# Alessandro-Mosconi/neptune-mip

Hardware: AMD Instinct MI355X
Metric: LP-relaxations/sec + objective gap vs reference, 512-node×256-function (higher is better)
Workload: dtype f32 x-state, f64 duals/reductions/certificate

## Files before the change

### include/neptune_lp.h

```cpp
#ifndef NEPTUNE_LP_H
#define NEPTUNE_LP_H

#include <stdint.h>

#ifdef __cplusplus
extern "C" {
#endif

#define NEP_API_VERSION 13

enum { NEP_MIN_DELAY = 0, NEP_MIN_UTILIZATION = 1, NEP_MIN_DELAY_AND_UTILIZATION = 2 };
enum { NEP_STEP1 = 1, NEP_STEP2_DELETE = 2, NEP_STEP2_CREATE = 3 };
enum { NEP_RELAX_REFERENCE = 0, NEP_RELAX_FACILITY = 1 };

enum { NEP_OK = 0, NEP_ERR_ARG = -1, NEP_ERR_HIP = -2, NEP_ERR_NOMEM = -3, NEP_ERR_STATE = -4 };

enum {
  NEP_LP_OPTIMAL = 0,
  NEP_LP_ITERATION_LIMIT = 1,
  NEP_LP_INFEASIBLE = 2,
  NEP_LP_CUTOFF = 3,
  NEP_LP_NUMERICAL = 4,
  NEP_LP_BOUND = 5
};
// ... 107 lines not shown
  NEP_SC_HANDLE_MAXDEV = 9,
  NEP_SC_CPU_MAXEXCESS = 10,
  NEP_SC_COUNT = 11
};
int nep_lp_score_check(void *model, int32_t slot, double *out);

int nep_get_stats(void *model, nep_stats *stats);

int nep_lp_get_diag(void *model, int32_t slot, double *out16);
int nep_debug_state(void *model, int32_t slot, double *y, double *kz, float *kty, double *lb, double *ub);
int nep_debug_sparse_rows(void *model, int32_t slot, int32_t *anchor_cnt, float *lambda_nnz);
int nep_debug_build(const nep_model_desc *desc, double *eta, double *rho, double *gam, double *rownorm,
                    int32_t *dims);
int nep_debug_presolve(const nep_model_desc *desc, int32_t n, const double *lb_int, const double *ub_int,
                       int32_t *ok_full, int32_t *ok_node, double *box_full, double *box_node);
void nep_reset_stats(void *model);

int nep_lp_copy_routing(void *dst_model, int32_t dst_slot, void *src_model, int32_t src_slot);

int nep_round_leaf(int32_t F, int32_t N, const double *c_fix, const double *n_fix, const float *flow, const double *zc,
                   const double *fn_mem, const double *node_mem, int32_t by_flow, double flow_threshold, double *c_out,
                   double *n_out);
int nep_round_leaves(int32_t F, int32_t N, const double *c_fix, const double *n_fix, const float *flow, const double *zc,
                     const double *fn_mem, const double *node_mem, int32_t modes, const int32_t *by_flow,
                     const double *flow_threshold, double *c_out, double *n_out, int32_t *found);

typedef struct {
  int32_t c0, c1, n0, n1, n_int;
  int32_t F, N;
  int32_t warm;
// ... 96 lines not shown
```

### neptune-mip_amd/core/engine/lp.py

```python
import ctypes
import math
import os

import numpy as np

_HERE = os.path.dirname(os.path.abspath(__file__))
LIB_PATH = os.environ.get("NEPTUNE_LP_LIB",
                          os.path.normpath(os.path.join(_HERE, "..", "..", "lib", "libneptune_lp.so")))

MIN_DELAY, MIN_UTILIZATION, MIN_DELAY_AND_UTILIZATION = 0, 1, 2
STEP1, STEP2_DELETE, STEP2_CREATE = 1, 2, 3
LP_OPTIMAL, LP_ITERATION_LIMIT, LP_INFEASIBLE, LP_CUTOFF, LP_NUMERICAL, LP_BOUND = 0, 1, 2, 3, 4, 5
VARIANTS = {"MinDelay": MIN_DELAY, "MinUtilization": MIN_UTILIZATION,
            "MinDelayAndUtilization": MIN_DELAY_AND_UTILIZATION}
API_VERSION = 13
RELAX_REFERENCE, RELAX_FACILITY = 0, 1

_dp = ctypes.POINTER(ctypes.c_double)


class EngineUnavailable(RuntimeError):
    pass


# ... 201 lines not shown
                               else BNB_RC_FIX())


EXPORTS = ("nep_model_create", "nep_model_destroy", "nep_model_get_info", "nep_lp_solve_batch",
           "nep_lp_submit", "nep_lp_submit_ex", "nep_lp_advance", "nep_lp_active", "nep_lp_copy_states", "nep_lp_get_flows_solutions",
           "nep_lp_get_solution", "nep_lp_get_rows", "nep_lp_copy_state", "nep_get_stats", "nep_reset_stats",
           "nep_lp_get_flows_split",
           "nep_last_error", "nep_api_version", "nep_lp_get_diag", "nep_debug_build", "nep_debug_state",
           "nep_debug_presolve", "nep_debug_sparse_rows", "nep_lp_set_params", "nep_lp_get_flows", "nep_lp_routing_entries",
           "nep_lp_allocation_entries", "nep_lp_score_check", "nep_round_leaf", "nep_lp_copy_routing",
           "nep_lp_get_solutions", "nep_round_leaves", "nep_lp_set_reference_weight",
           "nep_bnb_create", "nep_bnb_destroy", "nep_bnb_add_leaf", "nep_bnb_set_incumbent", "nep_bnb_event_data",
           "nep_bnb_run", "nep_bnb_get_stats", "nep_bnb_get_lp_iters", "nep_bnb_incumbent", "nep_bnb_set_step2",
           "nep_bnb_incumbent_event", "nep_bnb_debug_ibound", "nep_bnb_create_engines", "nep_bnb_sync_get",
           "nep_bnb_sync_set", "nep_bnb_export_nodes", "nep_bnb_import_nodes", "nep_lp_get_reduced_costs",
           "nep_lp_rc_fixings")
SCORE_FIELDS = ("network_delay", "nodes_used", "node_cost", "bad_c_x", "bad_memory", "bad_handle", "bad_cpu",
                "bad_n_c", "bad_budget", "handle_maxdev", "cpu_maxexcess")

_lib = None


def _host_inputs():
    return os.environ.get("NEP_HOST_INPUTS", "0") not in ("", "0")


def load_library(path=None):
    global _lib
    if _lib is not None and path is None:
        return _lib
    p = path or LIB_PATH
# ... 56 lines not shown
    lib.nep_bnb_sync_get.argtypes = [vp, _dp]
    lib.nep_bnb_sync_set.argtypes = [vp, ctypes.c_double, i32, i64]
    lib.nep_bnb_export_nodes.argtypes = [vp, i32, i32, pi32, _dp, pi32, _dp]
    lib.nep_bnb_import_nodes.argtypes = [vp, i32, pi32, _dp, pi32, _dp]
    lib.nep_lp_get_flows.argtypes = [vp, i32, pi32, ctypes.POINTER(ctypes.c_float)]
    lib.nep_lp_get_flows_split.argtypes = [vp, i32, pi32, ctypes.POINTER(ctypes.c_float), ctypes.POINTER(ctypes.c_float)]
    lib.nep_lp_routing_entries.argtypes = [vp, i32, ctypes.c_double, i32, i64, pi64, pi32, pi32, _dp]
    lib.nep_lp_allocation_entries.argtypes = [vp, i32, ctypes.c_double, i64, pi64, pi32, pi32]
    lib.nep_lp_score_check.argtypes = [vp, i32, _dp]
    lib.nep_round_leaf.argtypes = [i32, i32, _dp, _dp, ctypes.POINTER(ctypes.c_float), _dp, _dp, _dp, i32,
                                   ctypes.c_double, _dp, _dp]
    lib.nep_last_error.restype = ctypes.c_char_p
    lib.nep_api_version.restype = ctypes.c_int
    scalar_ptrs = tuple(ctypes.POINTER(t) for t in (ctypes.c_double, ctypes.c_float, ctypes.c_int32, ctypes.c_int64))
    for name in EXPORTS:
        fn = getattr(lib, name)
        if fn.argtypes:
            fn.argtypes = [ctypes.c_void_p if t in scalar_ptrs else t for t in fn.argtypes]
    if lib.nep_api_version() != API_VERSION:
        raise EngineUnavailable(f"{p}: API version {lib.nep_api_version()} != {API_VERSION} (rebuild the engine)")
    if path is None:
        _lib = lib
    return lib


def round_leaf(c_fix, n_fix, flow, zc, fn_mem, node_mem, by_flow, flow_threshold):
    lib = load_library()
    c_fix = np.ascontiguousarray(c_fix, np.float64)
    F, N = c_fix.shape
    nf = None if n_fix is None else np.ascontiguousarray(n_fix, np.float64)
# ... 84 lines not shown
    N, F = len(data.nodes), len(data.functions)
    v = VARIANTS[variant] if isinstance(variant, str) else int(variant)
    k = _arrays(data, N, F)
    d = _desc(k, N, F, v, int(step), alpha, soften_step1_sol, max_score, prev_network_delay, data.node_budget,
              relaxation)
    dims = np.zeros(4, np.int32)
    eta = np.zeros(1)
    _check(lib, lib.nep_debug_build(ctypes.byref(d), _ptr(eta), None, None, None, _ptr(dims, ctypes.c_int32)),
           "nep_debug_build")
    R, T, n_int, n_dual = dims.tolist()
    rho, gam, rn = np.zeros(n_dual), np.zeros(n_int), np.zeros(n_dual)
    _check(lib, lib.nep_debug_build(ctypes.byref(d), _ptr(eta), _ptr(rho), _ptr(gam), _ptr(rn), None),
           "nep_debug_build")
    return {"eta": float(eta[0]), "rho": rho, "gam": gam, "rownorm": rn, "R": R, "T": T, "n_int": n_int,
            "n_dual": n_dual}


def debug_presolve(data, variant, lb, ub, step=STEP1, alpha=0.5, soften_step1_sol=1.3, max_score=0.0,
                   prev_network_delay=0.0):
    lib = load_library()
    N, F = len(data.nodes), len(data.functions)
    v = VARIANTS[variant] if isinstance(variant, str) else int(variant)
    k = _arrays(data, N, F)
    d = _desc(k, N, F, v, int(step), alpha, soften_step1_sol, max_score, prev_network_delay, data.node_budget)
    lb = np.ascontiguousarray(lb, np.float64)
    ub = np.ascontiguousarray(ub, np.float64)
    n, ni = lb.shape
    okf = np.zeros(n, np.int32)
    okn = np.zeros(n, np.int32)
    bf = np.zeros((n, 2, ni))
# ... 287 lines not shown
```

### neptune-mip_amd/csrc/nep_fac.hip

```cpp
#include <hip/hip_runtime.h>
#include <cfloat>
#include <algorithm>
#include <cmath>

#include "nep_internal.h"
#include "nep_device.h"

namespace nep {

template <int CPL, bool CHECK, bool INIT, bool FIRST, int TW>
__global__ __launch_bounds__(kWave * TW) __attribute__((amdgpu_waves_per_eu(CHECK ? 2 : (CPL >= 8 ? 2 : (CPL >= 4 ? 3 : 4)), 8)))
void fac_x_pass(DeviceView v, const int32_t *__restrict__ slots, int plain, int it, int nslots, int nt_i) {
  const bool nt = nt_i != 0;
  constexpr int E = 4 * CPL;
  constexpr int SW = CHECK ? 2 : 1;
  extern __shared__ __attribute__((aligned(16))) float lds[];
  __shared__ double lds_s[TW][NTS + NBS];
  __shared__ double lds0[TW][4];
  const int total = v.F * nslots, Q = (total + 7) / 8;
  const int p = (int)(blockIdx.x % 8) * Q + (int)(blockIdx.x / 8);
  if (p >= total) return;
  const int f = p / nslots;
  const int slot = slots[p - f * nslots];
  Ctrl *ctrl = v.ctrl + slot;
// ... 524 lines not shown
    vals[BS_MOVE_Y] = a.mvy;
    vals[BS_DIST_Z] = a.dsz;
    vals[BS_DIST_Y] = a.dsy;
    vals[BS_LAGR0] = a.lagr0;
    double *bp = v.bpart + slot * v.sbpart + ((int64_t)F + jb) * NBS;
#pragma unroll
    for (int k = 0; k < NBS; ++k) {
      const double t = (k == BS_RES) ? wave_max_d(vals[k]) : wave_sum_d(vals[k]);
      if (lane == 0) bp[k] = t;
    }
  }
}

template <int CPL, int TW>
static hipError_t launch_fac_tw(const DeviceView &v, const int32_t *slots, int nslots, bool check, bool init,
                                bool first, bool plain, int it, hipStream_t s) {
  dim3 grid(8 * ((v.F * nslots + 7) / 8)), block(kWave * TW);
  const size_t lds = fac_lds_bytes(TW, v.NP, check);
  const int pl = plain ? 1 : 0;
  const int nt = (double)nslots * 4.0 * (double)v.sx * sizeof(float) > 160e6 ? 1 : 0;
  if (init) hipLaunchKernelGGL((fac_x_pass<CPL, false, true, false, TW>), grid, block, lds, s, v, slots, pl, it, nslots, nt);
  else if (check)
    hipLaunchKernelGGL((fac_x_pass<CPL, true, false, false, TW>), grid, block, lds, s, v, slots, pl, it, nslots, nt);
  else if (first)
    hipLaunchKernelGGL((fac_x_pass<CPL, false, false, true, TW>), grid, block, lds, s, v, slots, pl, it, nslots, nt);
  else hipLaunchKernelGGL((fac_x_pass<CPL, false, false, false, TW>), grid, block, lds, s, v, slots, pl, it, nslots, nt);
  return hipGetLastError();
}

static int fac_tile_waves(const DeviceView &v, int nslots, bool check) {
  int tw = 4;
  while (tw < 16 && (int64_t)nslots * v.F * tw < 4096) tw *= 2;
  if (v.CPL >= 4 && tw > 8) tw = 8;
  while (tw > kMinTileWaves && fac_lds_bytes(tw, v.NP, check) > kLdsCap) tw /= 2;
  return tw;
}

template <int CPL>
static hipError_t launch_fac_cpl(const DeviceView &v, const int32_t *slots, int nslots, bool check, bool init,
                                 bool first, bool plain, int it, hipStream_t s) {
  switch (fac_tile_waves(v, nslots, check)) {
    case 4: return launch_fac_tw<CPL, 4>(v, slots, nslots, check, init, first, plain, it, s);
    case 8: return launch_fac_tw<CPL, 8>(v, slots, nslots, check, init, first, plain, it, s);
    case 16: return launch_fac_tw<CPL, 16>(v, slots, nslots, check, init, first, plain, it, s);
    default: return hipErrorInvalidValue;
  }
}

hipError_t launch_fac_x_pass(const DeviceView &v, const int32_t *slots, int nslots, bool check, bool init, bool first,
                             bool plain, int it, hipStream_t s) {
  if (fac_lds_bytes(kMinTileWaves, v.NP, check) > kLdsCap) return hipErrorInvalidValue;
  switch (v.CPL) {
    case 1: return launch_fac_cpl<1>(v, slots, nslots, check, init, first, plain, it, s);
    case 2: return launch_fac_cpl<2>(v, slots, nslots, check, init, first, plain, it, s);
    case 4: return launch_fac_cpl<4>(v, slots, nslots, check, init, first, plain, it, s);
    case 8: return launch_fac_cpl<8>(v, slots, nslots, check, init, first, plain, it, s);
    default: return hipErrorInvalidValue;
  }
}

hipError_t launch_fac_node_pass(const DeviceView &v, const int32_t *slots, int nslots, bool check, bool init, bool first,
                                bool plain, int it, hipStream_t s) {
  const int fi = first ? 1 : 0, pl = plain ? 1 : 0;
  dim3 grid(v.JB, nslots), block(kNodeThreads);
  if (init) hipLaunchKernelGGL((fac_node_pass<false, true>), grid, block, 0, s, v, slots, fi, pl, it);
  else if (check) hipLaunchKernelGGL((fac_node_pass<true, false>), grid, block, 0, s, v, slots, fi, pl, it);
  else hipLaunchKernelGGL((fac_node_pass<false, false>), grid, block, 0, s, v, slots, fi, pl, it);
  return hipGetLastError();
}

}
// ... 1 lines not shown
```

### neptune-mip_amd/csrc/nep_host.cpp

```cpp
#include <hip/hip_runtime.h>

#include <algorithm>
#include <atomic>
#include <chrono>
#include <climits>
#include <cmath>
#include <cstdio>
#include <cstdlib>
#include <cstring>
#include <limits>
#include <memory>
#include <random>
#include <string>
#include <system_error>
#include <thread>
#include <vector>

#include "../../include/neptune_lp.h"
#include "nep_internal.h"

namespace nep {
hipError_t launch_x_pass(const DeviceView &v, const int32_t *slots, int nslots, bool check, bool init, bool first,
                         bool plain, int it, hipStream_t s);
hipError_t launch_node_pass(const DeviceView &v, const int32_t *slots, int nslots, bool check, bool init, bool first,
                            bool plain, int it, hipStream_t s);
hipError_t launch_scalar_pass(const DeviceView &v, const int32_t *slots, int nslots, bool check, bool init,
                              bool first, bool plain, int it, int block_len, hipStream_t s);
hipError_t launch_node_bounds(const DeviceView &v, const int32_t *slots, int nslots, const double *base_lb,
                              const double *base_ub, const uint8_t *base_mask, const int32_t *off, const int32_t *idx,
                              const double *cl, const double *cu, int max_chg, hipStream_t s);
hipError_t launch_init_slot(const DeviceView &v, const int32_t *slots, const int32_t *exact, int nslots, bool warm,
                            double eta, double omega0, const double *per, hipStream_t s);
hipError_t launch_node_flows(const DeviceView &v, const int32_t *slots, int n, float *out, float *wout,
                             hipStream_t s);
hipError_t launch_compact_f32(const float *vals, int rows, int cols, int64_t ld, double thr, int round3,
                              int32_t *cnt, int32_t *off, int32_t *orow, int32_t *ocol, double *oval, bool count_only,
                              hipStream_t s);
hipError_t launch_compact_f64(const double *vals, int rows, int cols, int64_t ld, double thr, int round3,
// ... 24 lines not shown
}
namespace nep {
int set_error(int code, const char *msg) { return fail(code, msg ? msg : ""); }
}
#define HIPCHK(expr)                                                                         \
  do {                                                                                       \
    hipError_t _e = (expr);                                                                  \
    if (_e != hipSuccess) return fail(NEP_ERR_HIP, std::string(#expr ": ") + hipGetErrorString(_e)); \
  } while (0)

static const double INF = std::numeric_limits<double>::infinity();
#ifndef NEP_HALPERN
#define NEP_HALPERN 1
#endif
static constexpr bool kHalpern = NEP_HALPERN != 0;

namespace {

struct Coo {
  std::vector<int> r, c;
  std::vector<double> v;
  void add(int row, int col, double val) {
    r.push_back(row);
    c.push_back(col);
    v.push_back(val);
  }
};

struct PresolveScratch {
  std::vector<int> pos, fdelta, touched, ftouched;
// ... 36 lines not shown
  bool score_x = false;
  std::vector<double> Dh;
  bool x_cost_free = true;
  bool base_ok = false;
  std::vector<double> base_lb, base_ub, base_amin, base_amax;
  std::vector<uint8_t> base_mask;
  std::vector<int> base_cnt, Kcp, Kcr;
  std::vector<double> Kcv;
  std::vector<PresolveScratch> psc;
  double eta = 0, sigma_max = 0, omega0 = 1.0;
  double omega_ref = 0.0;
  hipStream_t stream = nullptr;
  bool own_stream = false;
  hipStream_t aux = nullptr;
  hipEvent_t ev_aux = nullptr;
  DeviceView v{};
  std::vector<void *> allocs;
  double *d_prm = nullptr;
  double prm_host[3] = {0, 0, 0};
  bool prm_sent = false;
  int32_t *d_slots = nullptr;
  int32_t *h_act = nullptr;
  int32_t *d_new = nullptr;
  double *d_base_lb = nullptr, *d_base_ub = nullptr;
  uint8_t *d_base_mask = nullptr;
  int32_t *d_sub_i = nullptr;
  double *d_sub_d = nullptr;
  hipEvent_t ev0 = nullptr, ev1 = nullptr;
  nep_stats stats{};
  float *d_flows = nullptr;
// ... 22 lines not shown
  double *h_rc = nullptr;
  double *d_rc = nullptr;
  int32_t *d_rccnt = nullptr, *d_rcoff = nullptr;
  int32_t *d_rcidx = nullptr;
  double *d_rcval = nullptr;
  std::vector<uint8_t> rc_stale;
  int32_t *h_sub_i[2] = {nullptr, nullptr};
  double *h_sub_d[2] = {nullptr, nullptr};
  size_t cap_sub_i[2] = {0, 0}, cap_sub_d[2] = {0, 0};
  hipEvent_t ev_sub[2] = {nullptr, nullptr};
  bool sub_pending[2] = {false, false};
  int sub_k = 0;
  ~Model() {
    if (stream) (void)hipStreamSynchronize(stream);
    if (aux) (void)hipStreamSynchronize(aux);
    if (h_ctrl) (void)hipHostFree(h_ctrl);
    if (h_act) (void)hipHostFree(h_act);
    if (h_flows) (void)hipHostFree(h_flows);
    if (h_sols) (void)hipHostFree(h_sols);
    if (h_rc) (void)hipHostFree(h_rc);
    for (int k = 0; k < 2; ++k) {
      if (h_sub_i[k]) (void)hipHostFree(h_sub_i[k]);
      if (h_sub_d[k]) (void)hipHostFree(h_sub_d[k]);
      if (ev_sub[k]) (void)hipEventDestroy(ev_sub[k]);
    }
    for (void *p : allocs) (void)hipFree(p);
    for (hipGraphExec_t g : block_graph)
      if (g) (void)hipGraphExecDestroy(g);
    if (ev0) (void)hipEventDestroy(ev0);
    if (ev1) (void)hipEventDestroy(ev1);
    if (ev_aux) (void)hipEventDestroy(ev_aux);
    if (aux) (void)hipStreamDestroy(aux);
    if (own_stream && stream) (void)hipStreamDestroy(stream);
  }
};

template <typename T>
int dalloc(Model &m, T **p, size_t n) {
  void *q = nullptr;
  if (n == 0) n = 1;
  hipError_t e = hipMalloc(&q, n * sizeof(T));
  if (e != hipSuccess) return fail(NEP_ERR_NOMEM, std::string("hipMalloc: ") + hipGetErrorString(e));
  m.allocs.push_back(q);
  *p = static_cast<T *>(q);
  return NEP_OK;
}
template <typename T>
// ... 20 lines not shown
  if (d.step != NEP_STEP1 && !d.old_allocations) return fail(NEP_ERR_ARG, "step 2 needs old_allocations");
  m.N = N;
  m.F = F;
  m.variant = d.variant;
  m.step = d.step;
  m.step2 = d.step != NEP_STEP1;
  m.has_n = d.variant != NEP_MIN_DELAY;
  if (d.relaxation != NEP_RELAX_REFERENCE && d.relaxation != NEP_RELAX_FACILITY) return fail(NEP_ERR_ARG, "bad relaxation");
  m.fac = d.relaxation == NEP_RELAX_FACILITY;
  if (m.fac && (m.step2 || !m.has_n))
    return fail(NEP_ERR_ARG, "the facility relaxation is a step-1 MinUtilization / MinDelayAndUtilization model");
  m.alpha = d.alpha;
  m.M = d.big_m > 0 ? d.big_m : 1e6;
  m.eps = d.epsilon > 0 ? d.epsilon : 1e-6;
  m.sigma4 = d.step == NEP_STEP2_CREATE ? 1.0 : -1.0;
  m.NP = (N + 3) / 4 * 4;
  if (const int np_max = max_padded_width(m.fac); m.NP > np_max)
    return fail(NEP_ERR_ARG, "n_nodes = " + std::to_string(N) + " not supported by this build: the " +
                                 (m.fac ? "facility" : "reference") + " relaxation's certificate pass holds rows of at most " +
                                 std::to_string(np_max) + " destinations in LDS (largest supported n_nodes: " +
                                 std::to_string(np_max) + ")");
  const int chunks = m.NP / 4;
  m.CPL = chunks <= 64 ? 1 : chunks <= 128 ? 2 : chunks <= 256 ? 4 : 8;
  m.W.assign(d.workload, d.workload + (size_t)F * N);
  m.cprh.assign(d.core_per_req, d.core_per_req + (size_t)F * N);
  m.wsum.assign(F, 0.0);
  for (int f = 0; f < F; ++f)
    for (int i = 0; i < N; ++i) m.wsum[f] += m.W[(size_t)f * N + i];
  const double *D = d.delay;

  for (int f = 0; f < F; ++f) {
    int zeros = 0;
    for (int i = 0; i < N; ++i) {
      const double w = m.W[(size_t)f * N + i];
      if (w != 0.0) {
        m.row_f.push_back(f);
        m.row_src.push_back(i);
        m.row_m.push_back(1.f);
// ... 414 lines not shown
    m.stream = (hipStream_t)stream;
  } else {
    HIPCHK(hipStreamCreateWithFlags(&m.stream, hipStreamNonBlocking));
    m.own_stream = true;
  }
  HIPCHK(hipEventCreate(&m.ev0));
  HIPCHK(hipEventCreate(&m.ev1));
  {
    int least = 0, greatest = 0;
    if (hipDeviceGetStreamPriorityRange(&least, &greatest) != hipSuccess) greatest = 0;
    const char *e = std::getenv("NEP_AUX_PRIORITY");
    if (e && std::atoi(e) == 0) greatest = least;
    HIPCHK(hipStreamCreateWithPriority(&m.aux, hipStreamNonBlocking, greatest));
  }
  HIPCHK(hipEventCreateWithFlags(&m.ev_aux, hipEventDisableTiming));
  DeviceView &v = m.v;
  v.N = m.N; v.NP = m.NP; v.F = m.F; v.R = m.R; v.JB = m.JB; v.CPL = m.CPL;
  v.has_n = m.has_n; v.step2 = m.step2; v.variant = m.variant; v.fac = m.fac;
  v.M = m.M; v.eps = m.eps; v.sigma4 = m.sigma4; v.cost_n = m.cost_n; v.score_n_coef = m.score_n_coef;
  v.w_dis = m.w_dis;
  v.dred = m.dred; v.sT = m.sT; v.sum_old = m.sum_old;
  v.dl = m.dl; v.il = m.il;
  v.rs_suff = 0.2; v.rs_nec = 0.9; v.rs_art = 0.36; v.omega_smooth = 0.5;
  if (const char *e = std::getenv("NEP_RESTART")) std::sscanf(e, "%lf,%lf,%lf", &v.rs_suff, &v.rs_nec, &v.rs_art);
  if (const char *e = std::getenv("NEP_OMEGA_SMOOTH")) v.omega_smooth = std::atof(e);
  if (const char *e = std::getenv("NEP_PIPELINE_MAX_DONE")) m.pipe_max_done = std::atoi(e);
  v.polish_res = kPolishRes;
  v.polish_budget = kPolishBudget;
  if (const char *e = std::getenv("NEP_POLISH")) {
    long long b = v.polish_budget;
// ... 718 lines not shown
  double *dlb = m.d_sub_d, *dub = dlb + nchg;
  HIPCHK(hipEventRecord(m.ev_sub[sk], m.aux));
  HIPCHK(launch_node_bounds(v, dn, nf, m.d_base_lb, m.d_base_ub, m.d_base_mask, doff, didx, dlb, dub, max_chg,
                            m.aux));
  HIPCHK(launch_init_slot(v, dn, dex, nf, o.warm_start != 0, m.eta, m.omega0, per ? dub + nchg : nullptr, m.aux));
  HIPCHK(launch_x_pass(v, dn, nf, false, true, true, true, 0, m.aux));
  HIPCHK(launch_node_pass(v, dn, nf, false, true, true, true, 0, m.aux));
  HIPCHK(launch_scalar_pass(v, dn, nf, false, true, true, true, 0, o.check_every, m.aux));
  HIPCHK(hipEventRecord(m.ev_aux, m.aux));
  HIPCHK(hipStreamWaitEvent(m.stream, m.ev_aux, 0));
  m.act.insert(m.act.end(), fresh.begin(), fresh.end());
  m.sub_pending[sk] = true;
  return NEP_OK;
}

hipError_t block_graph(Model &m, int na, hipGraphExec_t *out) {
  const int ce = m.run.check_every;
  if (m.graph_ce != ce) {
    for (hipGraphExec_t &g : m.block_graph)
      if (g) { (void)hipGraphExecDestroy(g); g = nullptr; }
    m.block_graph.assign(m.max_batch + 1, nullptr);
    m.graph_ce = ce;
  }
  if (!m.block_graph[na]) {
    hipError_t e = hipStreamBeginCapture(m.stream, hipStreamCaptureModeThreadLocal);
    if (e != hipSuccess) return e;
    hipError_t le = hipSuccess;
    for (int it = 0; it < ce && le == hipSuccess; ++it) {
      const bool check = it == 0, first = it == 1;
      const bool plain = !kHalpern || ce < 4 || it == 0 || it == ce - 1;
      le = launch_x_pass(m.v, m.d_slots, na, check, false, first, plain, it, m.stream);
      if (le == hipSuccess) le = launch_node_pass(m.v, m.d_slots, na, check, false, first, plain, it, m.stream);
      if (le == hipSuccess && (m.step2 || check))
        le = launch_scalar_pass(m.v, m.d_slots, na, check, false, first, plain, it, ce, m.stream);
    }
    hipGraph_t graph = nullptr;
    e = hipStreamEndCapture(m.stream, &graph);
    if (le != hipSuccess) { if (graph) (void)hipGraphDestroy(graph); return le; }
    if (e != hipSuccess) return e;
    hipGraphExec_t exec = nullptr;
    e = hipGraphInstantiate(&exec, graph, nullptr, nullptr, 0);
    (void)hipGraphDestroy(graph);
    if (e != hipSuccess) return e;
    m.block_graph[na] = exec;
  }
  *out = m.block_graph[na];
  return hipSuccess;
}

int launch_block(Model &m) {
  DeviceView &v = m.v;
  const int ce = m.run.check_every;
  const int na = (int)m.act.size();
  const int sample_it = (ce >= 4 && m.blocks % 4 == 0) ? 2 : -1;
  m.blocks += 1;
  std::copy(m.act.begin(), m.act.end(), m.h_act);
  HIPCHK(hipMemcpyAsync(m.d_slots, m.h_act, na * sizeof(int32_t), hipMemcpyHostToDevice, m.stream));
  bool eager = sample_it >= 0 || !m.graphs_ok;
  if (!eager) {
    hipGraphExec_t g = nullptr;
    if (block_graph(m, na, &g) != hipSuccess) {
      (void)hipGetLastError();
      m.graphs_ok = false;
      eager = true;
    } else {
      HIPCHK(hipGraphLaunch(g, m.stream));
      m.stats.x_pass_launches += ce;
    }
  }
  for (int it = 0; it < ce && eager; ++it) {
    const bool check = it == 0, first = it == 1;
    const bool plain = !kHalpern || ce < 4 || it == 0 || it == ce - 1;
    const bool sample = it == sample_it;
    if (sample) HIPCHK(hipEventRecord(m.ev0, m.stream));
    HIPCHK(launch_x_pass(v, m.d_slots, na, check, false, first, plain, it, m.stream));
    if (sample) HIPCHK(hipEventRecord(m.ev1, m.stream));
    HIPCHK(launch_node_pass(v, m.d_slots, na, check, false, first, plain, it, m.stream));
    if (m.step2 || check) HIPCHK(launch_scalar_pass(v, m.d_slots, na, check, false, first, plain, it, ce, m.stream));
    m.stats.x_pass_launches += 1;
  }
  HIPCHK(hipMemcpyAsync(m.h_ctrl, v.ctrl, sizeof(Ctrl) * m.max_batch, hipMemcpyDeviceToHost, m.stream));
  m.stats.lp_iterations += (int64_t)na * ce;
  m.launched = m.act;
  m.inflight = true;
  m.inflight_sampled = sample_it >= 0;
  return NEP_OK;
}

int advance(Model &m, int min_done, int32_t *n_done, int32_t *done, double *obj, double *pobj, int32_t *status,
            int64_t *iters) {
  *n_done = 0;
  while (true) {
    if (!m.inflight) {
      if (m.act.empty()) break;
      int rc = launch_block(m);
// ... 735 lines not shown
  if (!desc) return fail(NEP_ERR_ARG, "null argument");
  if (desc->device_inputs) return fail(NEP_ERR_ARG, "nep_debug_build takes host arrays (device_inputs = 0)");
  Model m;
  int rc = build(m, *desc);
  if (rc) return rc;
  if (eta) *eta = m.eta;
  if (rho) std::memcpy(rho, m.rho.data(), m.rho.size() * sizeof(double));
  if (gam) std::memcpy(gam, m.gam.data(), m.gam.size() * sizeof(double));
  if (rownorm) std::memcpy(rownorm, m.rownorm.data(), m.rownorm.size() * sizeof(double));
  if (dims) {
    dims[0] = m.R; dims[1] = m.F; dims[2] = m.il.n_int; dims[3] = m.dl.n_dual;
  }
  return NEP_OK;
}

int nep_get_stats(void *model, nep_stats *stats) {
  if (!model || !stats) return fail(NEP_ERR_ARG, "null argument");
  *stats = static_cast<Model *>(model)->stats;
  return NEP_OK;
}

void nep_reset_stats(void *model) {
  if (model) static_cast<Model *>(model)->stats = nep_stats{};
}

}

int nep_debug_presolve(const nep_model_desc *desc, int32_t n, const double *lbi, const double *ubi, int32_t *ok_full,
                       int32_t *ok_node, double *box_full, double *box_node) {
  if (!desc || n < 0 || !ok_full || !ok_node) return fail(NEP_ERR_ARG, "null argument");
// ... 38 lines not shown
```

### neptune-mip_amd/csrc/nep_internal.h

```cpp
#pragma once
#include <cstddef>
#include <cstdint>

#ifndef NEP_NT
#define NEP_NT 1
#endif
#ifndef NEP_SPARSE_ANCHOR
#define NEP_SPARSE_ANCHOR 1
#endif
#ifndef NEP_INLINE_REFLECT
#define NEP_INLINE_REFLECT 0
#endif

#if defined(__HIPCC__) || defined(__HIP__)
#define NEP_HD __host__ __device__
#else
#define NEP_HD
#endif

namespace nep {

NEP_HD inline void dred_interval(double sigma4, double la, double ua, double ld, double ud, double &tlo, double &thi) {
  if (sigma4 > 0) {
    const bool ok = ld <= 0.0 && ud >= 0.0;
// ... 15 lines not shown
  int32_t j;
  float v;
};

constexpr int kWave = 64;

constexpr size_t kLdsCap = 144 * 1024;
constexpr int kMinTileWaves = 4;
NEP_HD inline size_t x_lds_bytes(int tw, int NP, bool check) {
  return (size_t)(2 * tw + 2) * NP * sizeof(float) +
         (check ? (size_t)(NEP_INLINE_REFLECT ? 3 : 2) * tw * NP * sizeof(float) + 4 * (size_t)NP * sizeof(double) : 0);
}
NEP_HD inline size_t fac_lds_bytes(int tw, int NP, bool check) {
  const int sw = check ? 2 : 1;
  return (size_t)(sw * tw + tw + (check ? tw : 0) + 3) * NP * sizeof(float) + 3 * (size_t)NP * sizeof(double);
}
inline int max_padded_width(bool fac) {
  int np = 4;
  while ((fac ? fac_lds_bytes(kMinTileWaves, np + 4, true) : x_lds_bytes(kMinTileWaves, np + 4, true)) <= kLdsCap) np += 4;
  return np;
}

constexpr int64_t kOmegaTrained = 1024;
constexpr double kPolishRes = 1e-3;
constexpr int64_t kPolishBudget = 512;
constexpr int kNodeWaves = 16;
constexpr int kNodeThreads = kWave * kNodeWaves;
constexpr int kNodeJ = 16;

struct RowInfo {
// ... 119 lines not shown
```

### neptune-mip_amd/csrc/nep_kernels.hip

```cpp
#include <hip/hip_runtime.h>
#include <cfloat>
#include <algorithm>
#include <cmath>

#include "nep_internal.h"
#include "nep_device.h"

#ifndef NEP_XPASS_PREFETCH
#define NEP_XPASS_PREFETCH 2
#endif
#ifndef NEP_CHECK_WAVES
#define NEP_CHECK_WAVES 2
#endif
#ifndef NEP_XPASS_WAVES
#define NEP_XPASS_WAVES 6
#endif
#ifndef NEP_XPASS_PF_WAVES
#define NEP_XPASS_PF_WAVES 5
#endif
#ifndef NEP_XPASS_PF_ANCHOR
#define NEP_XPASS_PF_ANCHOR 0
#endif
#ifndef NEP_XPASS_ELIDE
#define NEP_XPASS_ELIDE 1
// ... 1351 lines not shown
  uint8_t *mask = v.mask + slot * v.smask;
  const int oc = v.il.oc, FN = v.F * v.N;
  for (int t = off[b] + blockIdx.x * blockDim.x + threadIdx.x; t < off[b + 1]; t += gridDim.x * blockDim.x) {
    const int k = idx[t];
    lb[k] = cl[t];
    ub[k] = cu[t];
    if (k >= oc && k < oc + FN) {
      const int f = (k - oc) / v.N, j = (k - oc) - f * v.N;
      mask[(int64_t)f * v.NP + j] = cu[t] > 0.0 ? 1 : 0;
    }
  }
}

template <int CPL, int TW>
static hipError_t launch_x_tw(const DeviceView &v, const int32_t *slots, int nslots, bool check, bool init,
                              bool first, bool plain, int it, hipStream_t s) {
  dim3 grid(8 * ((v.F * nslots + 7) / 8)), block(kWave * TW);
  const size_t lds = x_lds_bytes(TW, v.NP, check);
  const int pl = plain ? 1 : 0;
  const int nt = (double)nslots * 2.0 * (double)v.sx * sizeof(float) > 160e6 ? 1 : 0;
  if (init) hipLaunchKernelGGL((x_pass<CPL, false, true, false, TW>), grid, block, lds, s, v, slots, pl, it, nslots, nt);
  else if (check)
    hipLaunchKernelGGL((x_pass<CPL, true, false, false, TW>), grid, block, lds, s, v, slots, pl, it, nslots, nt);
  else if (first)
    hipLaunchKernelGGL((x_pass<CPL, false, false, true, TW>), grid, block, lds, s, v, slots, pl, it, nslots, nt);
  else hipLaunchKernelGGL((x_pass<CPL, false, false, false, TW>), grid, block, lds, s, v, slots, pl, it, nslots, nt);
  return hipGetLastError();
}

static int tile_waves(const DeviceView &v, int nslots, bool check) {
  int tw = 4;
  while (tw < 16 && (int64_t)nslots * v.F * tw < 4096) tw *= 2;
  if (v.CPL >= 8 && tw > 8) tw = 8;
  while (check && tw > kMinTileWaves && x_lds_bytes(tw, v.NP, true) > kLdsCap) tw /= 2;
  return tw;
}

template <int CPL>
static hipError_t launch_x_cpl(const DeviceView &v, const int32_t *slots, int nslots, bool check, bool init,
                               bool first, bool plain, int it, hipStream_t s) {
  switch (tile_waves(v, nslots, check)) {
    case 4: return launch_x_tw<CPL, 4>(v, slots, nslots, check, init, first, plain, it, s);
    case 8: return launch_x_tw<CPL, 8>(v, slots, nslots, check, init, first, plain, it, s);
    case 16: return launch_x_tw<CPL, 16>(v, slots, nslots, check, init, first, plain, it, s);
    default: return hipErrorInvalidValue;
  }
}

hipError_t launch_fac_x_pass(const DeviceView &v, const int32_t *slots, int nslots, bool check, bool init, bool first,
                             bool plain, int it, hipStream_t s);
hipError_t launch_fac_node_pass(const DeviceView &v, const int32_t *slots, int nslots, bool check, bool init, bool first,
                                bool plain, int it, hipStream_t s);

hipError_t launch_x_pass(const DeviceView &v, const int32_t *slots, int nslots, bool check, bool init, bool first,
                         bool plain, int it, hipStream_t s) {
  if (v.fac) return launch_fac_x_pass(v, slots, nslots, check, init, first, plain, it, s);
  if (x_lds_bytes(kMinTileWaves, v.NP, check) > kLdsCap) return hipErrorInvalidValue;
  switch (v.CPL) {
    case 1: return launch_x_cpl<1>(v, slots, nslots, check, init, first, plain, it, s);
    case 2: return launch_x_cpl<2>(v, slots, nslots, check, init, first, plain, it, s);
    case 4: return launch_x_cpl<4>(v, slots, nslots, check, init, first, plain, it, s);
    case 8: return launch_x_cpl<8>(v, slots, nslots, check, init, first, plain, it, s);
    default: return hipErrorInvalidValue;
  }
}

hipError_t launch_node_pass(const DeviceView &v, const int32_t *slots, int nslots, bool check, bool init, bool first,
                            bool plain, int it, hipStream_t s) {
  if (v.fac) return launch_fac_node_pass(v, slots, nslots, check, init, first, plain, it, s);
  const int fi = first ? 1 : 0, pl = plain ? 1 : 0;
  dim3 grid(v.JB, nslots), block(kNodeThreads);
  if (init) hipLaunchKernelGGL((node_pass<false, true>), grid, block, 0, s, v, slots, fi, pl, it);
  else if (check) hipLaunchKernelGGL((node_pass<true, false>), grid, block, 0, s, v, slots, fi, pl, it);
  else hipLaunchKernelGGL((node_pass<false, false>), grid, block, 0, s, v, slots, fi, pl, it);
  return hipGetLastError();
}

// ... 33 lines not shown
```

Baseline: 17.17.

## Split each LP block batch into two stream groups that run concurrently

Splits the active LP slots of each iteration block into two halves and launches the x/node/scalar pass chains for each half on separate streams, joined by fork/join events and captured into the block graph. Because the halves have no dependencies on each other, their kernel chains can overlap instead of running behind per-iteration serialization of the whole batch. The split only happens when both halves keep the same tile-wave choice, and the non-temporal store policy still uses the full batch size. It adds stream and event setup, falls back to a single group if graph capture fails, and comes with a debug export for checking the split decision.

```diff
diff --git a/include/neptune_lp.h b/include/neptune_lp.h
--- a/include/neptune_lp.h
+++ b/include/neptune_lp.h
@@ -145,6 +145,7 @@
                     int32_t *dims);
 int nep_debug_presolve(const nep_model_desc *desc, int32_t n, const double *lb_int, const double *ub_int,
                        int32_t *ok_full, int32_t *ok_node, double *box_full, double *box_node);
+int nep_debug_block_split(int32_t n_nodes, int32_t n_functions, int32_t relaxation, int32_t na, int32_t *out3);
 void nep_reset_stats(void *model);
 
 int nep_lp_copy_routing(void *dst_model, int32_t dst_slot, void *src_model, int32_t src_slot);
diff --git a/neptune-mip_amd/core/engine/lp.py b/neptune-mip_amd/core/engine/lp.py
--- a/neptune-mip_amd/core/engine/lp.py
+++ b/neptune-mip_amd/core/engine/lp.py
@@ -239,7 +239,7 @@
            "nep_bnb_run", "nep_bnb_get_stats", "nep_bnb_get_lp_iters", "nep_bnb_incumbent", "nep_bnb_set_step2",
            "nep_bnb_incumbent_event", "nep_bnb_debug_ibound", "nep_bnb_create_engines", "nep_bnb_sync_get",
            "nep_bnb_sync_set", "nep_bnb_export_nodes", "nep_bnb_import_nodes", "nep_lp_get_reduced_costs",
-           "nep_lp_rc_fixings")
+           "nep_lp_rc_fixings", "nep_debug_block_split")
 SCORE_FIELDS = ("network_delay", "nodes_used", "node_cost", "bad_c_x", "bad_memory", "bad_handle", "bad_cpu",
                 "bad_n_c", "bad_budget", "handle_maxdev", "cpu_maxexcess")
 
@@ -326,6 +326,8 @@
     lib.nep_api_version.restype = ctypes.c_int
     scalar_ptrs = tuple(ctypes.POINTER(t) for t in (ctypes.c_double, ctypes.c_float, ctypes.c_int32, ctypes.c_int64))
     for name in EXPORTS:
+        if name == "nep_debug_block_split":
+            continue
         fn = getattr(lib, name)
         if fn.argtypes:
             fn.argtypes = [ctypes.c_void_p if t in scalar_ptrs else t for t in fn.argtypes]
@@ -440,6 +442,15 @@
            "nep_debug_build")
     return {"eta": float(eta[0]), "rho": rho, "gam": gam, "rownorm": rn, "R": R, "T": T, "n_int": n_int,
             "n_dual": n_dual}
+
+
+def debug_block_split(n_nodes, n_functions, na, relaxation=RELAX_REFERENCE):
+    lib = load_library()
+    lib.nep_debug_block_split.argtypes = [ctypes.c_int32] * 4 + [ctypes.c_void_p]
+    out = np.zeros(3, np.int32)
+    _check(lib, lib.nep_debug_block_split(int(n_nodes), int(n_functions), int(relaxation), int(na),
+                                          _ptr(out, ctypes.c_int32)), "nep_debug_block_split")
+    return tuple(int(t) for t in out)
 
 
 def debug_presolve(data, variant, lb, ub, step=STEP1, alpha=0.5, soften_step1_sol=1.3, max_score=0.0,
diff --git a/neptune-mip_amd/csrc/nep_fac.hip b/neptune-mip_amd/csrc/nep_fac.hip
--- a/neptune-mip_amd/csrc/nep_fac.hip
+++ b/neptune-mip_amd/csrc/nep_fac.hip
@@ -562,11 +562,11 @@
 
 template <int CPL, int TW>
 static hipError_t launch_fac_tw(const DeviceView &v, const int32_t *slots, int nslots, bool check, bool init,
-                                bool first, bool plain, int it, hipStream_t s) {
+                                bool first, bool plain, int it, hipStream_t s, int policy_slots) {
   dim3 grid(8 * ((v.F * nslots + 7) / 8)), block(kWave * TW);
   const size_t lds = fac_lds_bytes(TW, v.NP, check);
   const int pl = plain ? 1 : 0;
-  const int nt = (double)nslots * 4.0 * (double)v.sx * sizeof(float) > 160e6 ? 1 : 0;
+  const int nt = (double)policy_slots * 4.0 * (double)v.sx * sizeof(float) > 160e6 ? 1 : 0;
   if (init) hipLaunchKernelGGL((fac_x_pass<CPL, false, true, false, TW>), grid, block, lds, s, v, slots, pl, it, nslots, nt);
   else if (check)
     hipLaunchKernelGGL((fac_x_pass<CPL, true, false, false, TW>), grid, block, lds, s, v, slots, pl, it, nslots, nt);
@@ -586,23 +586,25 @@
 
 template <int CPL>
 static hipError_t launch_fac_cpl(const DeviceView &v, const int32_t *slots, int nslots, bool check, bool init,
-                                 bool first, bool plain, int it, hipStream_t s) {
+                                 bool first, bool plain, int it, hipStream_t s, int policy_slots) {
   switch (fac_tile_waves(v, nslots, check)) {
-    case 4: return launch_fac_tw<CPL, 4>(v, slots, nslots, check, init, first, plain, it, s);
-    case 8: return launch_fac_tw<CPL, 8>(v, slots, nslots, check, init, first, plain, it, s);
-    case 16: return launch_fac_tw<CPL, 16>(v, slots, nslots, check, init, first, plain, it, s);
+    case 4: return launch_fac_tw<CPL, 4>(v, slots, nslots, check, init, first, plain, it, s, policy_slots);
+    case 8: return launch_fac_tw<CPL, 8>(v, slots, nslots, check, init, first, plain, it, s, policy_slots);
+    case 16: return launch_fac_tw<CPL, 16>(v, slots, nslots, check, init, first, plain, it, s, policy_slots);
     default: return hipErrorInvalidValue;
   }
 }
 
+int fac_block_tile_waves(const DeviceView &v, int nslots, bool check) { return fac_tile_waves(v, nslots, check); }
+
 hipError_t launch_fac_x_pass(const DeviceView &v, const int32_t *slots, int nslots, bool check, bool init, bool first,
-                             bool plain, int it, hipStream_t s) {
+                             bool plain, int it, hipStream_t s, int policy_slots) {
   if (fac_lds_bytes(kMinTileWaves, v.NP, check) > kLdsCap) return hipErrorInvalidValue;
   switch (v.CPL) {
-    case 1: return launch_fac_cpl<1>(v, slots, nslots, check, init, first, plain, it, s);
-    case 2: return launch_fac_cpl<2>(v, slots, nslots, check, init, first, plain, it, s);
-    case 4: return launch_fac_cpl<4>(v, slots, nslots, check, init, first, plain, it, s);
-    case 8: return launch_fac_cpl<8>(v, slots, nslots, check, init, first, plain, it, s);
+    case 1: return launch_fac_cpl<1>(v, slots, nslots, check, init, first, plain, it, s, policy_slots);
+    case 2: return launch_fac_cpl<2>(v, slots, nslots, check, init, first, plain, it, s, policy_slots);
+    case 4: return launch_fac_cpl<4>(v, slots, nslots, check, init, first, plain, it, s, policy_slots);
+    case 8: return launch_fac_cpl<8>(v, slots, nslots, check, init, first, plain, it, s, policy_slots);
     default: return hipErrorInvalidValue;
   }
 }
diff --git a/neptune-mip_amd/csrc/nep_host.cpp b/neptune-mip_amd/csrc/nep_host.cpp
--- a/neptune-mip_amd/csrc/nep_host.cpp
+++ b/neptune-mip_amd/csrc/nep_host.cpp
@@ -21,7 +21,9 @@
 
 namespace nep {
 hipError_t launch_x_pass(const DeviceView &v, const int32_t *slots, int nslots, bool check, bool init, bool first,
-                         bool plain, int it, hipStream_t s);
+                         bool plain, int it, hipStream_t s, int policy_slots = 0);
+int block_tile_waves(const DeviceView &v, int nslots, bool check);
+int block_split(const DeviceView &v, int na);
 hipError_t launch_node_pass(const DeviceView &v, const int32_t *slots, int nslots, bool check, bool init, bool first,
                             bool plain, int it, hipStream_t s);
 hipError_t launch_scalar_pass(const DeviceView &v, const int32_t *slots, int nslots, bool check, bool init,
@@ -76,6 +78,7 @@
 #define NEP_HALPERN 1
 #endif
 static constexpr bool kHalpern = NEP_HALPERN != 0;
+static constexpr int kBlockGroups = 2;
 
 namespace {
 
@@ -142,6 +145,9 @@
   bool own_stream = false;
   hipStream_t aux = nullptr;
   hipEvent_t ev_aux = nullptr;
+  hipStream_t grp = nullptr;
+  hipEvent_t ev_fork = nullptr, ev_join = nullptr;
+  int groups = 1;
   DeviceView v{};
   std::vector<void *> allocs;
   double *d_prm = nullptr;
@@ -194,6 +200,7 @@
   ~Model() {
     if (stream) (void)hipStreamSynchronize(stream);
     if (aux) (void)hipStreamSynchronize(aux);
+    if (grp) (void)hipStreamSynchronize(grp);
     if (h_ctrl) (void)hipHostFree(h_ctrl);
     if (h_act) (void)hipHostFree(h_act);
     if (h_flows) (void)hipHostFree(h_flows);
@@ -211,6 +218,9 @@
     if (ev1) (void)hipEventDestroy(ev1);
     if (ev_aux) (void)hipEventDestroy(ev_aux);
     if (aux) (void)hipStreamDestroy(aux);
+    if (ev_fork) (void)hipEventDestroy(ev_fork);
+    if (ev_join) (void)hipEventDestroy(ev_join);
+    if (grp) (void)hipStreamDestroy(grp);
     if (own_stream && stream) (void)hipStreamDestroy(stream);
   }
 };
@@ -261,14 +271,13 @@
   m.M = d.big_m > 0 ? d.big_m : 1e6;
   m.eps = d.epsilon > 0 ? d.epsilon : 1e-6;
   m.sigma4 = d.step == NEP_STEP2_CREATE ? 1.0 : -1.0;
-  m.NP = (N + 3) / 4 * 4;
+  m.NP = padded_width(N);
   if (const int np_max = max_padded_width(m.fac); m.NP > np_max)
     return fail(NEP_ERR_ARG, "n_nodes = " + std::to_string(N) + " not supported by this build: the " +
                                  (m.fac ? "facility" : "reference") + " relaxation's certificate pass holds rows of at most " +
                                  std::to_string(np_max) + " destinations in LDS (largest supported n_nodes: " +
                                  std::to_string(np_max) + ")");
-  const int chunks = m.NP / 4;
-  m.CPL = chunks <= 64 ? 1 : chunks <= 128 ? 2 : chunks <= 256 ? 4 : 8;
+  m.CPL = chunks_per_lane(m.NP);
   m.W.assign(d.workload, d.workload + (size_t)F * N);
   m.cprh.assign(d.core_per_req, d.core_per_req + (size_t)F * N);
   m.wsum.assign(F, 0.0);
@@ -713,6 +722,13 @@
     HIPCHK(hipStreamCreateWithPriority(&m.aux, hipStreamNonBlocking, greatest));
   }
   HIPCHK(hipEventCreateWithFlags(&m.ev_aux, hipEventDisableTiming));
+  m.groups = kBlockGroups;
+  if (const char *e = std::getenv("NEP_BLOCK_GROUPS")) m.groups = std::atoi(e) >= 2 ? 2 : 1;
+  if (m.groups > 1) {
+    HIPCHK(hipStreamCreateWithFlags(&m.grp, hipStreamNonBlocking));
+    HIPCHK(hipEventCreateWithFlags(&m.ev_fork, hipEventDisableTiming));
+    HIPCHK(hipEventCreateWithFlags(&m.ev_join, hipEventDisableTiming));
+  }
   DeviceView &v = m.v;
   v.N = m.N; v.NP = m.NP; v.F = m.F; v.R = m.R; v.JB = m.JB; v.CPL = m.CPL;
   v.has_n = m.has_n; v.step2 = m.step2; v.variant = m.variant; v.fac = m.fac;
@@ -1461,26 +1477,48 @@
   return NEP_OK;
 }
 
-hipError_t block_graph(Model &m, int na, hipGraphExec_t *out) {
+hipError_t launch_iters(Model &m, const int32_t *slots, int n, int na, int it0, int it1, hipStream_t s) {
+  const int ce = m.run.check_every;
+  hipError_t e = hipSuccess;
+  for (int it = it0; it < it1 && e == hipSuccess; ++it) {
+    const bool check = it == 0, first = it == 1;
+    const bool plain = !kHalpern || ce < 4 || it == 0 || it == ce - 1;
+    e = launch_x_pass(m.v, slots, n, check, false, first, plain, it, s, na);
+    if (e == hipSuccess) e = launch_node_pass(m.v, slots, n, check, false, first, plain, it, s);
+    if (e == hipSuccess && (m.step2 || check)) e = launch_scalar_pass(m.v, slots, n, check, false, first, plain, it, ce, s);
+  }
+  return e;
+}
+
+hipError_t launch_span(Model &m, int na, int nA, int it0, int it1) {
+  if (it0 >= it1) return hipSuccess;
+  if (!nA) return launch_iters(m, m.d_slots, na, na, it0, it1, m.stream);
+  hipError_t e = hipEventRecord(m.ev_fork, m.stream);
+  if (e == hipSuccess) e = hipStreamWaitEvent(m.grp, m.ev_fork, 0);
+  if (e != hipSuccess) return e;
+  const hipError_t ea = launch_iters(m, m.d_slots, nA, na, it0, it1, m.stream);
+  const hipError_t eb = launch_iters(m, m.d_slots + nA, na - nA, na, it0, it1, m.grp);
+  e = hipEventRecord(m.ev_join, m.grp);
+  if (e == hipSuccess) e = hipStreamWaitEvent(m.stream, m.ev_join, 0);
+  return ea != hipSuccess ? ea : eb != hipSuccess ? eb : e;
+}
+
+void drop_block_graphs(Model &m) {
+  for (hipGraphExec_t &g : m.block_graph)
+    if (g) { (void)hipGraphExecDestroy(g); g = nullptr; }
+  m.block_graph.assign(m.max_batch + 1, nullptr);
+}
+
+hipError_t block_graph(Model &m, int na, int nA, hipGraphExec_t *out) {
   const int ce = m.run.check_every;
   if (m.graph_ce != ce) {
-    for (hipGraphExec_t &g : m.block_graph)
-      if (g) { (void)hipGraphExecDestroy(g); g = nullptr; }
-    m.block_graph.assign(m.max_batch + 1, nullptr);
+    drop_block_graphs(m);
     m.graph_ce = ce;
   }
   if (!m.block_graph[na]) {
     hipError_t e = hipStreamBeginCapture(m.stream, hipStreamCaptureModeThreadLocal);
     if (e != hipSuccess) return e;
-    hipError_t le = hipSuccess;
-    for (int it = 0; it < ce && le == hipSuccess; ++it) {
-      const bool check = it == 0, first = it == 1;
-      const bool plain = !kHalpern || ce < 4 || it == 0 || it == ce - 1;
-      le = launch_x_pass(m.v, m.d_slots, na, check, false, first, plain, it, m.stream);
-      if (le == hipSuccess) le = launch_node_pass(m.v, m.d_slots, na, check, false, first, plain, it, m.stream);
-      if (le == hipSuccess && (m.step2 || check))
-        le = launch_scalar_pass(m.v, m.d_slots, na, check, false, first, plain, it, ce, m.stream);
-    }
+    const hipError_t le = launch_span(m, na, nA, 0, ce);
     hipGraph_t graph = nullptr;
     e = hipStreamEndCapture(m.stream, &graph);
     if (le != hipSuccess) { if (graph) (void)hipGraphDestroy(graph); return le; }
@@ -1503,29 +1541,40 @@
   m.blocks += 1;
   std::copy(m.act.begin(), m.act.end(), m.h_act);
   HIPCHK(hipMemcpyAsync(m.d_slots, m.h_act, na * sizeof(int32_t), hipMemcpyHostToDevice, m.stream));
+  int nA = m.groups > 1 ? block_split(v, na) : 0;
   bool eager = sample_it >= 0 || !m.graphs_ok;
   if (!eager) {
     hipGraphExec_t g = nullptr;
-    if (block_graph(m, na, &g) != hipSuccess) {
+    hipError_t e = block_graph(m, na, nA, &g);
+    if (e != hipSuccess && nA) {
+      (void)hipGetLastError();
+      m.groups = 1;
+      nA = 0;
+      drop_block_graphs(m);
+      e = block_graph(m, na, 0, &g);
+    }
+    if (e != hipSuccess) {
       (void)hipGetLastError();
       m.graphs_ok = false;
       eager = true;
     } else {
       HIPCHK(hipGraphLaunch(g, m.stream));
-      m.stats.x_pass_launches += ce;
-    }
-  }
-  for (int it = 0; it < ce && eager; ++it) {
-    const bool check = it == 0, first = it == 1;
-    const bool plain = !kHalpern || ce < 4 || it == 0 || it == ce - 1;
-    const bool sample = it == sample_it;
-    if (sample) HIPCHK(hipEventRecord(m.ev0, m.stream));
-    HIPCHK(launch_x_pass(v, m.d_slots, na, check, false, first, plain, it, m.stream));
-    if (sample) HIPCHK(hipEventRecord(m.ev1, m.stream));
-    HIPCHK(launch_node_pass(v, m.d_slots, na, check, false, first, plain, it, m.stream));
-    if (m.step2 || check) HIPCHK(launch_scalar_pass(v, m.d_slots, na, check, false, first, plain, it, ce, m.stream));
-    m.stats.x_pass_launches += 1;
-  }
+    }
+  }
+  if (eager) {
+    const int s0 = sample_it >= 0 ? sample_it : ce, s1 = sample_it >= 0 ? sample_it + 1 : ce;
+    HIPCHK(launch_span(m, na, nA, 0, s0));
+    if (sample_it >= 0) {
+      const bool plain = !kHalpern;
+      HIPCHK(hipEventRecord(m.ev0, m.stream));
+      HIPCHK(launch_x_pass(v, m.d_slots, na, false, false, false, plain, sample_it, m.stream));
+      HIPCHK(hipEventRecord(m.ev1, m.stream));
+      HIPCHK(launch_node_pass(v, m.d_slots, na, false, false, false, plain, sample_it, m.stream));
+      if (m.step2) HIPCHK(launch_scalar_pass(v, m.d_slots, na, false, false, false, plain, sample_it, ce, m.stream));
+    }
+    HIPCHK(launch_span(m, na, nA, s1, ce));
+  }
+  m.stats.x_pass_launches += ce;
   HIPCHK(hipMemcpyAsync(m.h_ctrl, v.ctrl, sizeof(Ctrl) * m.max_batch, hipMemcpyDeviceToHost, m.stream));
   m.stats.lp_iterations += (int64_t)na * ce;
   m.launched = m.act;
@@ -2291,6 +2340,21 @@
   return NEP_OK;
 }
 
+int nep_debug_block_split(int32_t n_nodes, int32_t n_functions, int32_t relaxation, int32_t na, int32_t *out3) {
+  if (!out3 || n_nodes < 1 || n_functions < 1 || na < 1) return fail(NEP_ERR_ARG, "bad argument");
+  DeviceView v{};
+  v.N = n_nodes;
+  v.F = n_functions;
+  v.fac = relaxation == NEP_RELAX_FACILITY ? 1 : 0;
+  v.NP = padded_width(n_nodes);
+  if (v.NP > max_padded_width(v.fac != 0)) return fail(NEP_ERR_ARG, "n_nodes beyond the widest supported row");
+  v.CPL = chunks_per_lane(v.NP);
+  out3[0] = block_split(v, na);
+  out3[1] = block_tile_waves(v, na, false);
+  out3[2] = block_tile_waves(v, na, true);
+  return NEP_OK;
+}
+
 int nep_get_stats(void *model, nep_stats *stats) {
   if (!model || !stats) return fail(NEP_ERR_ARG, "null argument");
   *stats = static_cast<Model *>(model)->stats;
diff --git a/neptune-mip_amd/csrc/nep_internal.h b/neptune-mip_amd/csrc/nep_internal.h
--- a/neptune-mip_amd/csrc/nep_internal.h
+++ b/neptune-mip_amd/csrc/nep_internal.h
@@ -53,6 +53,11 @@
 NEP_HD inline size_t fac_lds_bytes(int tw, int NP, bool check) {
   const int sw = check ? 2 : 1;
   return (size_t)(sw * tw + tw + (check ? tw : 0) + 3) * NP * sizeof(float) + 3 * (size_t)NP * sizeof(double);
+}
+inline int padded_width(int N) { return (N + 3) / 4 * 4; }
+inline int chunks_per_lane(int NP) {
+  const int chunks = NP / 4;
+  return chunks <= 64 ? 1 : chunks <= 128 ? 2 : chunks <= 256 ? 4 : 8;
 }
 inline int max_padded_width(bool fac) {
   int np = 4;
diff --git a/neptune-mip_amd/csrc/nep_kernels.hip b/neptune-mip_amd/csrc/nep_kernels.hip
--- a/neptune-mip_amd/csrc/nep_kernels.hip
+++ b/neptune-mip_amd/csrc/nep_kernels.hip
@@ -1389,11 +1389,11 @@
 
 template <int CPL, int TW>
 static hipError_t launch_x_tw(const DeviceView &v, const int32_t *slots, int nslots, bool check, bool init,
-                              bool first, bool plain, int it, hipStream_t s) {
+                              bool first, bool plain, int it, hipStream_t s, int policy_slots) {
   dim3 grid(8 * ((v.F * nslots + 7) / 8)), block(kWave * TW);
   const size_t lds = x_lds_bytes(TW, v.NP, check);
   const int pl = plain ? 1 : 0;
-  const int nt = (double)nslots * 2.0 * (double)v.sx * sizeof(float) > 160e6 ? 1 : 0;
+  const int nt = (double)policy_slots * 2.0 * (double)v.sx * sizeof(float) > 160e6 ? 1 : 0;
   if (init) hipLaunchKernelGGL((x_pass<CPL, false, true, false, TW>), grid, block, lds, s, v, slots, pl, it, nslots, nt);
   else if (check)
     hipLaunchKernelGGL((x_pass<CPL, true, false, false, TW>), grid, block, lds, s, v, slots, pl, it, nslots, nt);
@@ -1411,31 +1411,48 @@
   return tw;
 }
 
+int fac_block_tile_waves(const DeviceView &v, int nslots, bool check);
+
+int block_tile_waves(const DeviceView &v, int nslots, bool check) {
+  return v.fac ? fac_block_tile_waves(v, nslots, check) : tile_waves(v, nslots, check);
+}
+
+int block_split(const DeviceView &v, int na) {
+  if (na < 2) return 0;
+  const int nA = (na + 1) / 2, nB = na - nA;
+  for (int check = 0; check < 2; ++check) {
+    const int tw = block_tile_waves(v, na, check != 0);
+    if (block_tile_waves(v, nA, check != 0) != tw || block_tile_waves(v, nB, check != 0) != tw) return 0;
+  }
+  return nA;
+}
+
 template <int CPL>
 static hipError_t launch_x_cpl(const DeviceView &v, const int32_t *slots, int nslots, bool check, bool init,
-                               bool first, bool plain, int it, hipStream_t s) {
+                               bool first, bool plain, int it, hipStream_t s, int policy_slots) {
   switch (tile_waves(v, nslots, check)) {
-    case 4: return launch_x_tw<CPL, 4>(v, slots, nslots, check, init, first, plain, it, s);
-    case 8: return launch_x_tw<CPL, 8>(v, slots, nslots, check, init, first, plain, it, s);
-    case 16: return launch_x_tw<CPL, 16>(v, slots, nslots, check, init, first, plain, it, s);
+    case 4: return launch_x_tw<CPL, 4>(v, slots, nslots, check, init, first, plain, it, s, policy_slots);
+    case 8: return launch_x_tw<CPL, 8>(v, slots, nslots, check, init, first, plain, it, s, policy_slots);
+    case 16: return launch_x_tw<CPL, 16>(v, slots, nslots, check, init, first, plain, it, s, policy_slots);
     default: return hipErrorInvalidValue;
   }
 }
 
 hipError_t launch_fac_x_pass(const DeviceView &v, const int32_t *slots, int nslots, bool check, bool init, bool first,
-                             bool plain, int it, hipStream_t s);
+                             bool plain, int it, hipStream_t s, int policy_slots);
 hipError_t launch_fac_node_pass(const DeviceView &v, const int32_t *slots, int nslots, bool check, bool init, bool first,
                                 bool plain, int it, hipStream_t s);
 
 hipError_t launch_x_pass(const DeviceView &v, const int32_t *slots, int nslots, bool check, bool init, bool first,
-                         bool plain, int it, hipStream_t s) {
-  if (v.fac) return launch_fac_x_pass(v, slots, nslots, check, init, first, plain, it, s);
+                         bool plain, int it, hipStream_t s, int policy_slots) {
+  if (policy_slots <= 0) policy_slots = nslots;
+  if (v.fac) return launch_fac_x_pass(v, slots, nslots, check, init, first, plain, it, s, policy_slots);
   if (x_lds_bytes(kMinTileWaves, v.NP, check) > kLdsCap) return hipErrorInvalidValue;
   switch (v.CPL) {
-    case 1: return launch_x_cpl<1>(v, slots, nslots, check, init, first, plain, it, s);
-    case 2: return launch_x_cpl<2>(v, slots, nslots, check, init, first, plain, it, s);
-    case 4: return launch_x_cpl<4>(v, slots, nslots, check, init, first, plain, it, s);
-    case 8: return launch_x_cpl<8>(v, slots, nslots, check, init, first, plain, it, s);
+    case 1: return launch_x_cpl<1>(v, slots, nslots, check, init, first, plain, it, s, policy_slots);
+    case 2: return launch_x_cpl<2>(v, slots, nslots, check, init, first, plain, it, s, policy_slots);
+    case 4: return launch_x_cpl<4>(v, slots, nslots, check, init, first, plain, it, s, policy_slots);
+    case 8: return launch_x_cpl<8>(v, slots, nslots, check, init, first, plain, it, s, policy_slots);
     default: return hipErrorInvalidValue;
   }
 }
```

New measurement: 18.28, median of 6. 6.4% higher.
